# QEDProtocol/plonky2.5

Measured on AMD Instinct MI355X. Metric: recursive proofs/sec (fib-64 p3-in-p2 circuit), higher is better.
Workload: dtype u64 (Goldilocks, p = 2^64 - 2^32 + 1); 1 GPU; batch of 256 independent fib-64 plonky3-verifier proofs per GPU (n = 2^16 rows x 135 wires, LDE 2^19), 1 GPU(s), replicas + RCCL gather; all_statuses_ok=True, gathered_complete_and_ok=True, head=

## Files before the change

### plonky2.5_amd/csrc/kernels_ntt.hip

```cpp
#include <mutex>
#include <set>
#include <tuple>
#include "kernels.h"
#include "ntt16.h"

constexpr int NTT_FACTOR_LOG = 16;

namespace p25 {

template <int G>
__device__ __forceinline__ void dif_group(u64* col, const u64* wl, int step, int l, int lstride, int s0) {
  constexpr int K = 1 << G;
  u64 x[K];
#pragma unroll
  for (int k = 0; k < K; k++) x[k] = col[k * step];
#pragma unroll
  for (int m = 0; m < G; m++) {
    constexpr int dummy = 0;
    (void)dummy;
    const int hk = K >> (m + 1);
#pragma unroll
    for (int k = 0; k < K; k++) {
      if (k & hk) continue;
      const int j = ((k & (hk - 1)) << lstride) + l;
      u64 sum, d;
      gl::bfly_nc(x[k], x[k + hk], false, sum, d);
      x[k] = sum;
      x[k + hk] = (hk == 1 && lstride == 0) ? d : gl::mul_nc(d, wl[j << (s0 + m)]);
    }
  }
#pragma unroll
  for (int k = 0; k < K; k++) col[k * step] = x[k];
}

template <bool INV>
__device__ __forceinline__ void dif16_group(u64* col, const u64* wl, int step, int l, int s0) {
  u64 x[16];
#pragma unroll
  for (int k = 0; k < 16; k++) x[k] = col[k * step];
  dft16<INV>(x);
  if (l != 0) {
#pragma unroll
    for (int k = 1; k < 16; k++) {
      const int f = ((k & 1) << 3) | ((k & 2) << 1) | ((k & 4) >> 1) | ((k & 8) >> 3);
      x[k] = gl::mul_nc(x[k], wl[(l * f) << s0]);
    }
  }
#pragma unroll
  for (int k = 0; k < 16; k++) col[k * step] = x[k];
}

template <bool INV, int NTH, int PRE>
__global__ __launch_bounds__(NTH) void k_ntt_tile(NttPass a) {
  P25_WAVE_PRIO(P25_PRIO_BULK);
  extern __shared__ u64 lds[];
  const int R = 1 << a.log_r, T = 1 << a.log_t;
  const int TP = T > 1 ? T + 1 : 1;
  u64* wl = lds + (size_t)R * TP;
  const u32 NT = 1u << a.log_nt;
  const int tid = threadIdx.x, nth = blockDim.x;
  const int wstride_log = a.log_n_table - a.log_r;
  for (int k = tid; k < (a.full_table ? R : R / 2); k += nth) wl[k] = a.pow_table[(size_t)k << wstride_log];
  const u32 L = blockIdx.x;
  const u32 m = L >> a.log_g;
  const u32 tiles_g = a.n_tiles >> a.log_g;
  const u32 coset = m % a.n_cosets;
  const u32 r = m / a.n_cosets;
  const u32 tile = (r % tiles_g) * (1u << a.log_g) + (L & ((1u << a.log_g) - 1u));
  const u32 poly = r / tiles_g;
  const u32 tg0 = tile * T;
  const u64* in = a.in + (size_t)poly * a.in_poly_stride;
  u64* out = a.out + (size_t)poly * a.out_poly_stride + a.coset_out_off[coset];
  const u64* pre = PRE == 1 ? a.pre + ((size_t)coset << (a.log_r + a.log_nt)) : nullptr;
  const u64* pre_i = PRE == 2 ? a.pre_i + ((size_t)coset << a.log_r) : nullptr;
  const u64 pre_tv = PRE == 2 ? a.pre_t[((size_t)coset << a.log_nt) + tg0 + (tid & (T - 1))] : 1;
  auto in_slot = [&](int e, size_t& addr, int& slot, int& ii) {
    int t, i;
    if (a.in_kind == 0) {
      t = e & (T - 1);
      i = e >> a.log_t;
      u32 ipos = a.in_br_i ? gl::bitrev(i, a.log_r) : i;
      addr = (size_t)(tg0 + t) + (size_t)ipos * NT;
    } else {
      int off = e & (R - 1);
      t = e >> a.log_r;
      i = a.in_br_i ? (int)gl::bitrev(off, a.log_r) : off;
      u32 trow = a.in_br_t ? gl::bitrev(tg0 + t, a.log_nt) : tg0 + t;
      addr = (size_t)trow * R + off;
    }
    slot = i * TP + t;
    ii = i;
  };
  constexpr int LB = 8;
  int e = tid;
  for (; e + (LB - 1) * nth < T * R; e += LB * nth) {
    u64 xv[LB], pv[LB];
    int slot[LB];
#pragma unroll
    for (int k = 0; k < LB; k++) {
      size_t addr;
      int ii;
      in_slot(e + k * nth, addr, slot[k], ii);
      xv[k] = in[addr];
      if constexpr (PRE == 1) pv[k] = pre[addr];
      else if constexpr (PRE == 2) pv[k] = pre_i[ii];
      else pv[k] = 1;
    }
#pragma unroll
    for (int k = 0; k < LB; k++) {
      if constexpr (PRE == 1) lds[slot[k]] = gl::mul_nc(xv[k], pv[k]);
      else if constexpr (PRE == 2) lds[slot[k]] = gl::mul_nc(gl::mul_nc(xv[k], pre_tv), pv[k]);
      else lds[slot[k]] = xv[k];
    }
  }
  for (; e < T * R; e += nth) {
    size_t addr;
    int slot, ii;
    in_slot(e, addr, slot, ii);
    u64 x = in[addr];
    if constexpr (PRE == 1) x = gl::mul_nc(x, pre[addr]);
    if constexpr (PRE == 2) x = gl::mul_nc(gl::mul_nc(x, pre_tv), pre_i[ii]);
    lds[slot] = x;
  }
  __syncthreads();

  for (int s0 = 0; s0 < a.log_r;) {
    const int g = a.log_r - s0 < 4 ? a.log_r - s0 : 4;
    const int lstride = a.log_r - s0 - g;
    const int items = T << (a.log_r - g);
    for (int b = tid; b < items; b += nth) {
      const int t = b & (T - 1), q = b >> a.log_t;
      const int l = q & ((1 << lstride) - 1), h = q >> lstride;
      u64* col = lds + ((h << (a.log_r - s0)) + l) * TP + t;
      switch (g) {
        case 4:
          if (a.full_table)
            dif16_group<INV>(col, wl, TP << lstride, l, s0);
          else
            dif_group<4>(col, wl, TP << lstride, l, lstride, s0);
          break;
        case 3: dif_group<3>(col, wl, TP << lstride, l, lstride, s0); break;
        case 2: dif_group<2>(col, wl, TP << lstride, l, lstride, s0); break;
        default: dif_group<1>(col, wl, TP << lstride, l, lstride, s0); break;
      }
    }
    __syncthreads();
    s0 += g;
  }

  auto out_slot = [&](int e, size_t& addr, int& slot, u32& tw, u32& j) {
    int t, q;
    if (a.out_kind == 0) {
      t = e & (T - 1);
      q = e >> a.log_t;
      j = gl::bitrev(q, a.log_r);
      u32 ipos = a.out_br_i ? (u32)q : j;
      addr = (size_t)(tg0 + t) + (size_t)ipos * NT;
    } else {
      int off = e & (R - 1);
      t = e >> a.log_r;
      q = a.out_br_i ? off : (int)gl::bitrev(off, a.log_r);
      j = gl::bitrev(q, a.log_r);
      u32 trow = a.out_br_t ? gl::bitrev(tg0 + t, a.log_nt) : tg0 + t;
      addr = (size_t)trow * R + off;
    }
    slot = q * TP + t;
    tw = (u32)(tg0 + t);
  };
  int eo = tid;
  if (a.use_twiddle && !a.post_t) {
    for (; eo + (LB - 1) * nth < T * R; eo += LB * nth) {
      u64 wv[LB], xv[LB];
      size_t addr[LB];
#pragma unroll
      for (int k = 0; k < LB; k++) {
        int slot;
        u32 tw, j;
        out_slot(eo + k * nth, addr[k], slot, tw, j);
        wv[k] = a.pow_table[(size_t)tw * j];
        xv[k] = lds[slot];
      }
#pragma unroll
      for (int k = 0; k < LB; k++) {
        const u64 y = gl::mul_nc(xv[k], wv[k]);
        out[addr[k]] = a.lazy_out ? y : gl::canon(y);
      }
    }
  }
  for (; eo < T * R; eo += nth) {
    size_t addr;
    int slot;
    u32 tw, j;
    out_slot(eo, addr, slot, tw, j);
    u64 x = lds[slot];
    if (a.use_twiddle) x = gl::mul_nc(x, a.pow_table[(size_t)tw * j]);
    if (a.post_t) x = gl::mul_nc(x, gl::mul_nc(a.post_t[tw], a.post_i[j]));
    out[addr] = a.lazy_out ? x : gl::canon(x);
  }
}

static size_t tile_lds_bytes(int log_r, int log_t) {
  const size_t R = (size_t)1 << log_r, T = (size_t)1 << log_t, TP = T > 1 ? T + 1 : 1;
  return (R * TP + (log_r <= 10 ? R : R / 2)) * sizeof(u64);
}

void launch_ntt_pass(const NttPass& p, int n_polys, int n_cosets, hipStream_t st) {
  NttPass q = p;
  q.full_table = p.log_r <= 10;
  size_t lds = tile_lds_bytes(p.log_r, p.log_t);
  q.n_tiles = 1u << (p.log_nt - p.log_t);
  q.n_cosets = (uint32_t)n_cosets;
  q.log_g = 0;
  while (q.log_g < 3 && (2u << q.log_g) <= q.n_tiles) q.log_g++;
  const dim3 grid(q.n_tiles * (uint32_t)n_polys * (uint32_t)n_cosets);
  const bool wide = p.log_r + p.log_t >= 13;
  const int pre_mode = q.pre ? 1 : (q.pre_t ? 2 : 0);
  auto launch = [&](auto kernel, int nth) {
    if (lds > 64 * 1024) {
      static std::mutex mu;
      static std::set<std::pair<int, const void*>> allowed;
      int dev = 0;
      P25_HIP(hipGetDevice(&dev));
      std::lock_guard<std::mutex> lk(mu);
      if (allowed.insert({dev, (const void*)kernel}).second)
        P25_HIP(hipFuncSetAttribute((const void*)kernel, hipFuncAttributeMaxDynamicSharedMemorySize, 160 * 1024));
    }
    hipLaunchKernelGGL(kernel, grid, dim3(nth), lds, st, q);
  };
#define P25_NTT_LAUNCH(INV, NTH)                                                            \
  switch (pre_mode) {                                                                       \
    case 1: launch(k_ntt_tile<INV, NTH, 1>, NTH); break;                                    \
    case 2: launch(k_ntt_tile<INV, NTH, 2>, NTH); break;                                    \
    default: launch(k_ntt_tile<INV, NTH, 0>, NTH); break;                                   \
  }
  if (wide) {
    if (q.inverse) { P25_NTT_LAUNCH(true, 512) } else { P25_NTT_LAUNCH(false, 512) }
  } else {
    if (q.inverse) { P25_NTT_LAUNCH(true, 256) } else { P25_NTT_LAUNCH(false, 256) }
  }
#undef P25_NTT_LAUNCH
}

static int pick_log_t(int log_r, int log_nt, bool strided) {
  int lt = 12 - log_r;
  if (strided)
    for (int w = 4; w > lt; w--)
      if (tile_lds_bytes(log_r, w) <= 79 * 1024) {
        lt = w;
        break;
      }
  if (!strided && log_r == 10) lt = 3;
  if (lt > 4) lt = 4;
  if (lt > log_nt) lt = log_nt;
  if (lt < 0) lt = 0;
  return lt;
}

void ntt_inverse_then_lde(NttTables& tb, const u64* d_vals, size_t val_stride, u64* d_tmp, size_t tmp_stride, u64* d_coeffs,
                          size_t coeff_stride, u64* d_lde, size_t lde_stride, int log_n, int rate_bits, int n_polys, u64 shift,
                          hipStream_t st) {
  ntt_inverse(tb, d_vals, val_stride, false, d_tmp, tmp_stride, d_coeffs, coeff_stride, log_n, n_polys, 1, st);
  ntt_lde_bitrev(tb, d_coeffs, coeff_stride, d_lde, lde_stride, log_n, rate_bits, n_polys, shift, st);
}

const u64* NttTables::upload(const std::vector<u64>& host) {
  owned_.emplace_back(host.size());
  u64* d = owned_.back().p;
  P25_HIP(hipMemcpy(d, host.data(), host.size() * sizeof(u64), hipMemcpyHostToDevice));
  return d;
}
const u64* NttTables::pow_table(int log_n, bool inverse) {
  auto key = std::make_pair(log_n, inverse);
  auto it = pow_.find(key);
  if (it != pow_.end()) return it->second;
  u64 w = gl::root_of_unity(log_n);
  if (inverse) w = gl::inv(w);
  std::vector<u64> h((size_t)1 << log_n);
  u64 x = 1;
  for (auto& v : h) {
    v = x;
    x = gl::mul(x, w);
  }
  u64* d = const_cast<u64*>(upload(h));
  pow_[key] = d;
  return d;
}
const u64* NttTables::geom_table(u64 first, u64 ratio, size_t len) {
  auto key = std::make_tuple(first, ratio, len);
  auto it = geom_.find(key);
  if (it != geom_.end()) return it->second;
  std::vector<u64> h(len);
  u64 x = first;
  for (auto& v : h) {
    v = x;
    x = gl::mul(x, ratio);
  }
  u64* d = const_cast<u64*>(upload(h));
  geom_[key] = d;
  return d;
}

static void split(int log_n, int& log_r1, int& log_r2) {
  if (log_n <= 10) {
    log_r1 = 0;
    log_r2 = log_n;
  } else {
    log_r2 = log_n / 2;
    log_r1 = log_n - log_r2;
  }
  if (log_r1 > 11 || log_r2 > 11) throw std::runtime_error("NTT size above 2^22 not supported");
}

void ntt_inverse(NttTables& tb, const u64* d_in, size_t in_stride, bool in_bitrev, u64* d_tmp,
                 size_t tmp_stride, u64* d_out, size_t out_stride, int log_n, int n_polys,
                 u64 coset_shift, hipStream_t st) {
  int l1, l2;
  split(log_n, l1, l2);
  const u64* pw = tb.pow_table(log_n, true);
  u64 n_inv = gl::inv((u64)1 << log_n);
  u64 s_inv = gl::inv(coset_shift);
  NttPass p{};
  p.pow_table = pw;
  p.log_n_table = log_n;
  p.inverse = 1;
  if (l1 == 0) {
    p.in = d_in; p.out = d_out;
    p.in_poly_stride = in_stride; p.out_poly_stride = out_stride;
    p.log_r = l2; p.log_nt = 0; p.log_t = 0;
    p.in_kind = 1; p.in_br_i = in_bitrev;
    p.out_kind = 1; p.out_br_i = 0;
    p.post_t = tb.geom_table(n_inv, 1, 1);
    p.post_i = tb.geom_table(1, s_inv, (size_t)1 << l2);
    launch_ntt_pass(p, n_polys, 1, st);
    return;
  }
  p.in = d_in; p.out = d_tmp;
  p.in_poly_stride = in_stride; p.out_poly_stride = tmp_stride;
  p.log_r = l2; p.log_nt = l1; p.log_t = pick_log_t(l2, l1, true);
  if (in_bitrev) { p.in_kind = 1; p.in_br_t = 1; p.in_br_i = 1; } else { p.in_kind = 0; }
  p.out_kind = 0; p.out_br_i = 0;
  p.use_twiddle = 1;
  p.lazy_out = 1;
  launch_ntt_pass(p, n_polys, 1, st);
  NttPass q{};
  q.pow_table = pw; q.log_n_table = log_n;
  q.inverse = 1;
  q.in = d_tmp; q.out = d_out;
  q.in_poly_stride = tmp_stride; q.out_poly_stride = out_stride;
  q.log_r = l1; q.log_nt = l2; q.log_t = pick_log_t(l1, l2, false);
  q.in_kind = 1;
  q.out_kind = 0; q.out_br_i = 0;
  q.post_t = tb.geom_table(n_inv, s_inv, (size_t)1 << l2);
  q.post_i = tb.geom_table(1, gl::pow(s_inv, (u64)1 << l2), (size_t)1 << l1);
  launch_ntt_pass(q, n_polys, 1, st);
}

void ntt_lde_bitrev(NttTables& tb, const u64* d_coeffs, size_t coeff_stride, u64* d_lde,
                    size_t lde_stride, int log_n, int rate_bits, int n_polys, u64 shift,
                    hipStream_t st) {
  int l1, l2;
  split(log_n, l1, l2);
  const int nc = 1 << rate_bits;
  if (nc > 8) throw std::runtime_error("rate_bits > 3 not supported");
  const size_t n = (size_t)1 << log_n;
  const u64* pw = tb.pow_table(log_n, false);
  const u64 w_big = gl::root_of_unity(log_n + rate_bits);
  auto& cache = tb.coset_cache();
  const bool factored = l1 != 0 && log_n > NTT_FACTOR_LOG;
  auto key = std::make_tuple(factored ? -log_n : log_n, rate_bits, shift);
  auto it = cache.find(key);
  if (it == cache.end()) {
    std::vector<u64> h;
    if (!factored) {
      h.resize((size_t)nc * n);
      for (int c = 0; c < nc; c++) {
        u64 sc = gl::mul(shift, gl::pow(w_big, c));
        u64 x = 1;
        for (size_t k = 0; k < n; k++) {
          h[(size_t)c * n + k] = x;
          x = gl::mul(x, sc);
        }
      }
    } else {
      const size_t R1 = (size_t)1 << l1, R2 = (size_t)1 << l2;
      h.resize((size_t)nc * (R1 + R2));
      for (int c = 0; c < nc; c++) {
        const u64 sc = gl::mul(shift, gl::pow(w_big, c)), sc_r1 = gl::pow(sc, R1);
        u64 x = 1;
        for (size_t k = 0; k < R1; k++) {
          h[(size_t)c * R1 + k] = x;
          x = gl::mul(x, sc);
        }
        x = 1;
        for (size_t k = 0; k < R2; k++) {
          h[(size_t)nc * R1 + (size_t)c * R2 + k] = x;
          x = gl::mul(x, sc_r1);
        }
      }
    }
    it = cache.emplace(key, tb.upload(h)).first;
  }

  NttPass p{};
  p.pow_table = pw; p.log_n_table = log_n;
  p.in = d_coeffs; p.out = d_lde;
  p.in_poly_stride = coeff_stride; p.out_poly_stride = lde_stride;
  for (int c = 0; c < nc; c++) p.coset_out_off[c] = (size_t)gl::bitrev(c, rate_bits) * n;
  if (factored) {
    p.pre_t = it->second;
    p.pre_i = it->second + ((size_t)nc << l1);
  } else {
    p.pre = it->second;
  }
  if (l1 == 0) {
    p.log_r = l2; p.log_nt = 0; p.log_t = 0;
    p.in_kind = 1; p.out_kind = 1; p.out_br_i = 1;
    launch_ntt_pass(p, n_polys, nc, st);
    return;
  }
  p.log_r = l2; p.log_nt = l1; p.log_t = pick_log_t(l2, l1, true);
  p.in_kind = 0; p.out_kind = 0; p.out_br_i = 1;
  p.use_twiddle = 1;
  p.lazy_out = 1;
  launch_ntt_pass(p, n_polys, nc, st);
  NttPass q{};
  q.pow_table = pw; q.log_n_table = log_n;
  q.in = d_lde; q.out = d_lde;
  q.in_poly_stride = lde_stride; q.out_poly_stride = lde_stride;
  q.log_r = l1; q.log_nt = l2 + rate_bits; q.log_t = pick_log_t(l1, l2 + rate_bits, false);
  q.in_kind = 1; q.out_kind = 1; q.out_br_i = 1;
  launch_ntt_pass(q, n_polys, 1, st);
}

}
```

Baseline: 135.8 proofs/s.

## Specialize NTT tile kernel by access form with incremental index cursors

Replaces the runtime-branched index computation in the NTT tile kernel with template-specialized load/store cursors per input/output layout and multiplier mode, using 32-bit offsets and incremental stepping. Adds a fully compile-time stage network for the common log_r=8, log_t=4 shape, and precomputes twiddle pointers in the radix-16 group. The goal is to cut integer address arithmetic, branches and 64-bit index math in a hot kernel. In exchange it brings template bloat, 32-bit offsets that could overflow on large buffers, and a runtime throw for any pass form not in the list.

```diff
diff --git a/plonky2.5_amd/csrc/kernels_ntt.hip b/plonky2.5_amd/csrc/kernels_ntt.hip
--- a/plonky2.5_amd/csrc/kernels_ntt.hip
+++ b/plonky2.5_amd/csrc/kernels_ntt.hip
@@ -3,6 +3,7 @@
 #include <tuple>
 #include "kernels.h"
 #include "ntt16.h"
+#include "ntt_index.h"
 
 constexpr int NTT_FACTOR_LOG = 16;
 
@@ -33,169 +34,172 @@
   for (int k = 0; k < K; k++) col[k * step] = x[k];
 }
 
-template <bool INV>
+template <bool INV, int STEP>
 __device__ __forceinline__ void dif16_group(u64* col, const u64* wl, int step, int l, int s0) {
+  const int st = STEP > 0 ? STEP : step;
   u64 x[16];
 #pragma unroll
-  for (int k = 0; k < 16; k++) x[k] = col[k * step];
+  for (int k = 0; k < 16; k++) x[k] = col[k * st];
   dft16<INV>(x);
   if (l != 0) {
+    const u64* wf[16];
+    wf[0] = wl;
+#pragma unroll
+    for (int f = 1; f < 16; f++) wf[f] = wf[f - 1] + (l << s0);
 #pragma unroll
     for (int k = 1; k < 16; k++) {
       const int f = ((k & 1) << 3) | ((k & 2) << 1) | ((k & 4) >> 1) | ((k & 8) >> 3);
-      x[k] = gl::mul_nc(x[k], wl[(l * f) << s0]);
-    }
-  }
-#pragma unroll
-  for (int k = 0; k < 16; k++) col[k * step] = x[k];
-}
-
-template <bool INV, int NTH, int PRE>
+      x[k] = gl::mul_nc(x[k], *wf[f]);
+    }
+  }
+#pragma unroll
+  for (int k = 0; k < 16; k++) col[k * st] = x[k];
+}
+
+template <bool INV, bool FULL, int STEP>
+__device__ __forceinline__ void dif_stages(u64* lds, const u64* wl, int log_r, int log_t, int s0, int g, int tid, int nth) {
+  const int T = 1 << log_t, TP = (int)nttix::row_pitch(log_t);
+  const int lstride = log_r - s0 - g;
+  const int items = T << (log_r - g);
+  for (int b = tid; b < items; b += nth) {
+    const int t = b & (T - 1), q = b >> log_t;
+    const int l = q & ((1 << lstride) - 1), h = q >> lstride;
+    u64* col = lds + ((h << (log_r - s0)) + l) * TP + t;
+    switch (g) {
+      case 4:
+        if (FULL)
+          dif16_group<INV, STEP>(col, wl, TP << lstride, l, s0);
+        else
+          dif_group<4>(col, wl, TP << lstride, l, lstride, s0);
+        break;
+      case 3: dif_group<3>(col, wl, TP << lstride, l, lstride, s0); break;
+      case 2: dif_group<2>(col, wl, TP << lstride, l, lstride, s0); break;
+      default: dif_group<1>(col, wl, TP << lstride, l, lstride, s0); break;
+    }
+  }
+  __syncthreads();
+}
+template <bool INV, int NTH, int LR, int LT, int S0>
+__device__ __forceinline__ void dif_network_static(u64* lds, const u64* wl, int tid) {
+  if constexpr (S0 < LR) {
+    constexpr int g = LR - S0 < 4 ? LR - S0 : 4;
+    constexpr int TP = LT ? (1 << LT) + 1 : 1;
+    dif_stages<INV, (LR <= 10), (g == 4 ? TP << (LR - S0 - g) : 0)>(lds, wl, LR, LT, S0, g, tid, NTH);
+    dif_network_static<INV, NTH, LR, LT, S0 + g>(lds, wl, tid);
+  }
+}
+
+__device__ __forceinline__ u64 ld_w(const u64* base, u32 woff) {
+  return *reinterpret_cast<const u64*>(reinterpret_cast<const char*>(base) + (woff << 3));
+}
+__device__ __forceinline__ void st_w(u64* base, u32 woff, u64 v) {
+  *reinterpret_cast<u64*>(reinterpret_cast<char*>(base) + (woff << 3)) = v;
+}
+
+template <bool INV, int NTH, int PRE, int IN, int OUT, int MUL, bool LAZY, int LR, int LT>
 __global__ __launch_bounds__(NTH) void k_ntt_tile(NttPass a) {
   P25_WAVE_PRIO(P25_PRIO_BULK);
   extern __shared__ u64 lds[];
-  const int R = 1 << a.log_r, T = 1 << a.log_t;
-  const int TP = T > 1 ? T + 1 : 1;
+  const int log_r = LR >= 0 ? LR : a.log_r, log_t = LT >= 0 ? LT : a.log_t;
+  const int R = 1 << log_r, T = 1 << log_t;
+  const int TP = (int)nttix::row_pitch(log_t);
+  const int TR = T * R;
   u64* wl = lds + (size_t)R * TP;
-  const u32 NT = 1u << a.log_nt;
-  const int tid = threadIdx.x, nth = blockDim.x;
-  const int wstride_log = a.log_n_table - a.log_r;
-  for (int k = tid; k < (a.full_table ? R : R / 2); k += nth) wl[k] = a.pow_table[(size_t)k << wstride_log];
-  const u32 L = blockIdx.x;
-  const u32 m = L >> a.log_g;
-  const u32 tiles_g = a.n_tiles >> a.log_g;
-  const u32 coset = m % a.n_cosets;
-  const u32 r = m / a.n_cosets;
-  const u32 tile = (r % tiles_g) * (1u << a.log_g) + (L & ((1u << a.log_g) - 1u));
-  const u32 poly = r / tiles_g;
-  const u32 tg0 = tile * T;
-  const u64* in = a.in + (size_t)poly * a.in_poly_stride;
-  u64* out = a.out + (size_t)poly * a.out_poly_stride + a.coset_out_off[coset];
-  const u64* pre = PRE == 1 ? a.pre + ((size_t)coset << (a.log_r + a.log_nt)) : nullptr;
-  const u64* pre_i = PRE == 2 ? a.pre_i + ((size_t)coset << a.log_r) : nullptr;
-  const u64 pre_tv = PRE == 2 ? a.pre_t[((size_t)coset << a.log_nt) + tg0 + (tid & (T - 1))] : 1;
-  auto in_slot = [&](int e, size_t& addr, int& slot, int& ii) {
-    int t, i;
-    if (a.in_kind == 0) {
-      t = e & (T - 1);
-      i = e >> a.log_t;
-      u32 ipos = a.in_br_i ? gl::bitrev(i, a.log_r) : i;
-      addr = (size_t)(tg0 + t) + (size_t)ipos * NT;
-    } else {
-      int off = e & (R - 1);
-      t = e >> a.log_r;
-      i = a.in_br_i ? (int)gl::bitrev(off, a.log_r) : off;
-      u32 trow = a.in_br_t ? gl::bitrev(tg0 + t, a.log_nt) : tg0 + t;
-      addr = (size_t)trow * R + off;
-    }
-    slot = i * TP + t;
-    ii = i;
+  const int tid = threadIdx.x;
+  const int wstride_log = a.log_n_table - log_r;
+  const bool full_table = log_r <= 10;
+  for (int k = tid; k < (full_table ? R : R / 2); k += NTH) wl[k] = a.pow_table[(size_t)k << wstride_log];
+  const nttix::BlockId blk = nttix::decode_block(blockIdx.x, a.log_g, a.n_tiles, a.n_cosets);
+  const nttix::Tile tile{log_r, log_t, a.log_nt, blk.tile << log_t};
+  const u64* in = a.in + (size_t)blk.poly * a.in_poly_stride;
+  u64* out = a.out + (size_t)blk.poly * a.out_poly_stride + a.coset_out_off[blk.coset];
+  const u64* pre = PRE == 1 ? a.pre + ((size_t)blk.coset << (log_r + a.log_nt)) : nullptr;
+  const u64* pre_i = PRE == 2 ? a.pre_i + ((size_t)blk.coset << log_r) : nullptr;
+  const u64 pre_tv = PRE == 2 ? a.pre_t[((size_t)blk.coset << a.log_nt) + tile.tg0 + (tid & (T - 1))] : 1;
+  constexpr int LB = 8;
+  {
+    nttix::LoadCursor<IN> lc;
+    lc.init(tile, tid, NTH);
+    int e = tid;
+    for (; e + (LB - 1) * NTH < TR; e += LB * NTH) {
+      u64 xv[LB], pv[LB];
+      u32 slot[LB];
+#pragma unroll
+      for (int k = 0; k < LB; k++) {
+        const u32 g = lc.goff();
+        slot[k] = lc.slot();
+        xv[k] = ld_w(in, g);
+        if constexpr (PRE == 1) pv[k] = ld_w(pre, g);
+        else if constexpr (PRE == 2) pv[k] = pre_i[lc.idx()];
+        else pv[k] = 1;
+        lc.next();
+      }
+#pragma unroll
+      for (int k = 0; k < LB; k++) {
+        if constexpr (PRE == 1) lds[slot[k]] = gl::mul_nc(xv[k], pv[k]);
+        else if constexpr (PRE == 2) lds[slot[k]] = gl::mul_nc(gl::mul_nc(xv[k], pre_tv), pv[k]);
+        else lds[slot[k]] = xv[k];
+      }
+    }
+    for (; e < TR; e += NTH) {
+      const u32 g = lc.goff();
+      u64 x = ld_w(in, g);
+      if constexpr (PRE == 1) x = gl::mul_nc(x, ld_w(pre, g));
+      if constexpr (PRE == 2) x = gl::mul_nc(gl::mul_nc(x, pre_tv), pre_i[lc.idx()]);
+      lds[lc.slot()] = x;
+      lc.next();
+    }
+  }
+  __syncthreads();
+
+  if constexpr (LR >= 0) {
+    dif_network_static<INV, NTH, LR, LT, 0>(lds, wl, tid);
+  } else {
+    for (int s0 = 0; s0 < log_r;) {
+      const int g = log_r - s0 < 4 ? log_r - s0 : 4;
+      if (full_table)
+        dif_stages<INV, true, 0>(lds, wl, log_r, log_t, s0, g, tid, NTH);
+      else
+        dif_stages<INV, false, 0>(lds, wl, log_r, log_t, s0, g, tid, NTH);
+      s0 += g;
+    }
+  }
+
+  nttix::StoreCursor<OUT> sc;
+  sc.init(tile, tid, NTH);
+  constexpr bool T_KIND = OUT == nttix::OUT_T || OUT == nttix::OUT_T_BR;
+  const u64 post_tv = (MUL == nttix::MUL_POST && T_KIND) ? a.post_t[sc.tw()] : 1;
+  auto multiplier = [&](u64& w, u64& pt) {
+    if constexpr (MUL == nttix::MUL_TWIDDLE) w = ld_w(a.pow_table, __umul24(sc.tw(), sc.j()));
+    if constexpr (MUL == nttix::MUL_POST) {
+      w = a.post_i[sc.j()];
+      pt = T_KIND ? post_tv : a.post_t[sc.tw()];
+    }
   };
-  constexpr int LB = 8;
-  int e = tid;
-  for (; e + (LB - 1) * nth < T * R; e += LB * nth) {
-    u64 xv[LB], pv[LB];
-    int slot[LB];
-#pragma unroll
-    for (int k = 0; k < LB; k++) {
-      size_t addr;
-      int ii;
-      in_slot(e + k * nth, addr, slot[k], ii);
-      xv[k] = in[addr];
-      if constexpr (PRE == 1) pv[k] = pre[addr];
-      else if constexpr (PRE == 2) pv[k] = pre_i[ii];
-      else pv[k] = 1;
-    }
-#pragma unroll
-    for (int k = 0; k < LB; k++) {
-      if constexpr (PRE == 1) lds[slot[k]] = gl::mul_nc(xv[k], pv[k]);
-      else if constexpr (PRE == 2) lds[slot[k]] = gl::mul_nc(gl::mul_nc(xv[k], pre_tv), pv[k]);
-      else lds[slot[k]] = xv[k];
-    }
-  }
-  for (; e < T * R; e += nth) {
-    size_t addr;
-    int slot, ii;
-    in_slot(e, addr, slot, ii);
-    u64 x = in[addr];
-    if constexpr (PRE == 1) x = gl::mul_nc(x, pre[addr]);
-    if constexpr (PRE == 2) x = gl::mul_nc(gl::mul_nc(x, pre_tv), pre_i[ii]);
-    lds[slot] = x;
-  }
-  __syncthreads();
-
-  for (int s0 = 0; s0 < a.log_r;) {
-    const int g = a.log_r - s0 < 4 ? a.log_r - s0 : 4;
-    const int lstride = a.log_r - s0 - g;
-    const int items = T << (a.log_r - g);
-    for (int b = tid; b < items; b += nth) {
-      const int t = b & (T - 1), q = b >> a.log_t;
-      const int l = q & ((1 << lstride) - 1), h = q >> lstride;
-      u64* col = lds + ((h << (a.log_r - s0)) + l) * TP + t;
-      switch (g) {
-        case 4:
-          if (a.full_table)
-            dif16_group<INV>(col, wl, TP << lstride, l, s0);
-          else
-            dif_group<4>(col, wl, TP << lstride, l, lstride, s0);
-          break;
-        case 3: dif_group<3>(col, wl, TP << lstride, l, lstride, s0); break;
-        case 2: dif_group<2>(col, wl, TP << lstride, l, lstride, s0); break;
-        default: dif_group<1>(col, wl, TP << lstride, l, lstride, s0); break;
-      }
-    }
-    __syncthreads();
-    s0 += g;
-  }
-
-  auto out_slot = [&](int e, size_t& addr, int& slot, u32& tw, u32& j) {
-    int t, q;
-    if (a.out_kind == 0) {
-      t = e & (T - 1);
-      q = e >> a.log_t;
-      j = gl::bitrev(q, a.log_r);
-      u32 ipos = a.out_br_i ? (u32)q : j;
-      addr = (size_t)(tg0 + t) + (size_t)ipos * NT;
-    } else {
-      int off = e & (R - 1);
-      t = e >> a.log_r;
-      q = a.out_br_i ? off : (int)gl::bitrev(off, a.log_r);
-      j = gl::bitrev(q, a.log_r);
-      u32 trow = a.out_br_t ? gl::bitrev(tg0 + t, a.log_nt) : tg0 + t;
-      addr = (size_t)trow * R + off;
-    }
-    slot = q * TP + t;
-    tw = (u32)(tg0 + t);
+  auto finish = [&](u64 x, u64 w, u64 pt) {
+    if constexpr (MUL == nttix::MUL_TWIDDLE) x = gl::mul_nc(x, w);
+    if constexpr (MUL == nttix::MUL_POST) x = gl::mul_nc(x, gl::mul_nc(pt, w));
+    return LAZY ? x : gl::canon(x);
   };
   int eo = tid;
-  if (a.use_twiddle && !a.post_t) {
-    for (; eo + (LB - 1) * nth < T * R; eo += LB * nth) {
-      u64 wv[LB], xv[LB];
-      size_t addr[LB];
-#pragma unroll
-      for (int k = 0; k < LB; k++) {
-        int slot;
-        u32 tw, j;
-        out_slot(eo + k * nth, addr[k], slot, tw, j);
-        wv[k] = a.pow_table[(size_t)tw * j];
-        xv[k] = lds[slot];
-      }
-#pragma unroll
-      for (int k = 0; k < LB; k++) {
-        const u64 y = gl::mul_nc(xv[k], wv[k]);
-        out[addr[k]] = a.lazy_out ? y : gl::canon(y);
-      }
-    }
-  }
-  for (; eo < T * R; eo += nth) {
-    size_t addr;
-    int slot;
-    u32 tw, j;
-    out_slot(eo, addr, slot, tw, j);
-    u64 x = lds[slot];
-    if (a.use_twiddle) x = gl::mul_nc(x, a.pow_table[(size_t)tw * j]);
-    if (a.post_t) x = gl::mul_nc(x, gl::mul_nc(a.post_t[tw], a.post_i[j]));
-    out[addr] = a.lazy_out ? x : gl::canon(x);
+  for (; eo + (LB - 1) * NTH < TR; eo += LB * NTH) {
+    u64 wv[LB], ptv[LB], xv[LB];
+    u32 g[LB];
+#pragma unroll
+    for (int k = 0; k < LB; k++) {
+      g[k] = sc.goff();
+      multiplier(wv[k], ptv[k]);
+      xv[k] = lds[sc.slot()];
+      sc.next();
+    }
+#pragma unroll
+    for (int k = 0; k < LB; k++) st_w(out, g[k], finish(xv[k], wv[k], ptv[k]));
+  }
+  for (; eo < TR; eo += NTH) {
+    u64 w = 1, pt = 1;
+    multiplier(w, pt);
+    st_w(out, sc.goff(), finish(lds[sc.slot()], w, pt));
+    sc.next();
   }
 }
 
@@ -205,6 +209,7 @@
 }
 
 void launch_ntt_pass(const NttPass& p, int n_polys, int n_cosets, hipStream_t st) {
+  using namespace nttix;
   NttPass q = p;
   q.full_table = p.log_r <= 10;
   size_t lds = tile_lds_bytes(p.log_r, p.log_t);
@@ -214,6 +219,7 @@
   while (q.log_g < 3 && (2u << q.log_g) <= q.n_tiles) q.log_g++;
   const dim3 grid(q.n_tiles * (uint32_t)n_polys * (uint32_t)n_cosets);
   const bool wide = p.log_r + p.log_t >= 13;
+  const bool hot = p.log_r == 8 && p.log_t == 4;
   const int pre_mode = q.pre ? 1 : (q.pre_t ? 2 : 0);
   auto launch = [&](auto kernel, int nth) {
     if (lds > 64 * 1024) {
@@ -227,18 +233,36 @@
     }
     hipLaunchKernelGGL(kernel, grid, dim3(nth), lds, st, q);
   };
-#define P25_NTT_LAUNCH(INV, NTH)                                                            \
-  switch (pre_mode) {                                                                       \
-    case 1: launch(k_ntt_tile<INV, NTH, 1>, NTH); break;                                    \
-    case 2: launch(k_ntt_tile<INV, NTH, 2>, NTH); break;                                    \
-    default: launch(k_ntt_tile<INV, NTH, 0>, NTH); break;                                   \
-  }
-  if (wide) {
-    if (q.inverse) { P25_NTT_LAUNCH(true, 512) } else { P25_NTT_LAUNCH(false, 512) }
-  } else {
-    if (q.inverse) { P25_NTT_LAUNCH(true, 256) } else { P25_NTT_LAUNCH(false, 256) }
-  }
-#undef P25_NTT_LAUNCH
+  int in = -1, out = -1;
+  if (p.in_kind == 0 && !p.in_br_i) in = IN_T;
+  if (p.in_kind == 1 && !p.in_br_t && !p.in_br_i) in = IN_I;
+  if (p.in_kind == 1 && p.in_br_i && (p.in_br_t || p.log_nt == 0)) in = IN_I_BR;
+  if (!p.out_br_t) out = p.out_kind == 0 ? (p.out_br_i ? OUT_T_BR : OUT_T) : (p.out_br_i ? OUT_I_BR : OUT_I);
+  const int mul = p.post_t ? MUL_POST : (p.use_twiddle ? MUL_TWIDDLE : MUL_NONE);
+  const bool both = p.post_t && p.use_twiddle;
+#define P25_NTT_FORM(INV, PRE, IN, OUT, MUL, LAZY, WIDE, HOT)                                                         \
+  if (!both && (bool)q.inverse == INV && pre_mode == PRE && in == IN && out == OUT && mul == MUL && (bool)q.lazy_out == LAZY && \
+      (WIDE || !wide)) {                                                                                              \
+    if (wide) {                                                                                                       \
+      if constexpr (WIDE) launch(k_ntt_tile<INV, 512, PRE, IN, OUT, MUL, LAZY, -1, -1>, 512);                         \
+    } else if (HOT && hot) {                                                                                          \
+      if constexpr (HOT) launch(k_ntt_tile<INV, 256, PRE, IN, OUT, MUL, LAZY, 8, 4>, 256);                            \
+    } else {                                                                                                          \
+      launch(k_ntt_tile<INV, 256, PRE, IN, OUT, MUL, LAZY, -1, -1>, 256);                                             \
+    }                                                                                                                 \
+    return;                                                                                                           \
+  }
+  P25_NTT_FORM(true, 0, IN_T, OUT_T, MUL_TWIDDLE, true, true, true)
+  P25_NTT_FORM(true, 0, IN_I_BR, OUT_T, MUL_TWIDDLE, true, true, false)
+  P25_NTT_FORM(true, 0, IN_I, OUT_T, MUL_POST, false, true, true)
+  P25_NTT_FORM(true, 0, IN_I, OUT_I, MUL_POST, false, false, false)
+  P25_NTT_FORM(true, 0, IN_I_BR, OUT_I, MUL_POST, false, false, false)
+  P25_NTT_FORM(false, 1, IN_T, OUT_T_BR, MUL_TWIDDLE, true, true, true)
+  P25_NTT_FORM(false, 2, IN_T, OUT_T_BR, MUL_TWIDDLE, true, true, false)
+  P25_NTT_FORM(false, 0, IN_I, OUT_I_BR, MUL_NONE, false, true, true)
+  P25_NTT_FORM(false, 1, IN_I, OUT_I_BR, MUL_NONE, false, false, false)
+#undef P25_NTT_FORM
+  throw std::runtime_error("NTT pass of a form the library has no kernel for");
 }
 
 static int pick_log_t(int log_r, int log_nt, bool strided) {
diff --git a/plonky2.5_amd/csrc/ntt_index.h b/plonky2.5_amd/csrc/ntt_index.h
--- /dev/null
+++ b/plonky2.5_amd/csrc/ntt_index.h
@@ -0,0 +1,140 @@
+#pragma once
+#include <stdint.h>
+
+#if defined(__HIPCC__)
+#define NTTIX_HD __host__ __device__ __forceinline__
+#else
+#define NTTIX_HD inline
+#endif
+
+namespace p25 {
+namespace nttix {
+
+enum In : int {
+  IN_T = 0,
+  IN_I = 1,
+  IN_I_BR = 2,
+};
+enum Out : int {
+  OUT_T = 0,
+  OUT_T_BR = 1,
+  OUT_I = 2,
+  OUT_I_BR = 3,
+};
+enum Mul : int {
+  MUL_NONE = 0,
+  MUL_TWIDDLE = 1,
+  MUL_POST = 2,
+};
+
+struct Tile {
+  int log_r, log_t, log_nt;
+  uint32_t tg0;
+};
+
+NTTIX_HD uint32_t brev(uint32_t x, int bits) {
+#if defined(__HIP_DEVICE_COMPILE__)
+  return bits ? (__brev(x) >> (32 - bits)) : 0;
+#else
+  uint32_t r = 0;
+  for (int b = 0; b < bits; b++) r |= ((x >> b) & 1u) << (bits - 1 - b);
+  return r;
+#endif
+}
+NTTIX_HD uint32_t row_pitch(int log_t) { return log_t ? (1u << log_t) + 1u : 1u; }
+
+struct BlockId {
+  uint32_t tile, poly, coset;
+};
+NTTIX_HD BlockId decode_block(uint32_t L, uint32_t log_g, uint32_t n_tiles, uint32_t n_cosets) {
+  const uint32_t m = L >> log_g, tiles_g = n_tiles >> log_g;
+  const uint32_t r = m / n_cosets;
+  return BlockId{(r % tiles_g) * (1u << log_g) + (L & ((1u << log_g) - 1u)), r / tiles_g, m % n_cosets};
+}
+
+template <int IN>
+struct LoadCursor {
+  uint32_t g, s, i;
+  uint32_t dg, ds, di;
+  uint32_t e, de, base;
+  int log_r, log_nt;
+  uint32_t tp, tg0;
+
+  NTTIX_HD void init(const Tile& a, uint32_t tid, uint32_t nth) {
+    log_r = a.log_r, log_nt = a.log_nt, tp = row_pitch(a.log_t), tg0 = a.tg0;
+    if constexpr (IN == IN_T) {
+      const uint32_t t = tid & ((1u << a.log_t) - 1u);
+      i = tid >> a.log_t, di = nth >> a.log_t;
+      g = tg0 + t + (i << log_nt), dg = di << log_nt;
+      s = i * tp + t, ds = di * tp;
+    } else {
+      e = tid, de = nth, base = tg0 << log_r;
+    }
+  }
+  NTTIX_HD void next() {
+    if constexpr (IN == IN_T) g += dg, s += ds, i += di;
+    else e += de;
+  }
+  NTTIX_HD uint32_t idx() const {
+    if constexpr (IN == IN_T) return i;
+    const uint32_t off = e & ((1u << log_r) - 1u);
+    return IN == IN_I_BR ? brev(off, log_r) : off;
+  }
+  NTTIX_HD uint32_t slot() const {
+    if constexpr (IN == IN_T) return s;
+    return idx() * tp + (e >> log_r);
+  }
+  NTTIX_HD uint32_t goff() const {
+    if constexpr (IN == IN_T) return g;
+    if constexpr (IN == IN_I) return base + e;
+    return (brev(tg0 + (e >> log_r), log_nt) << log_r) + (e & ((1u << log_r) - 1u));
+  }
+};
+
+template <int OUT>
+struct StoreCursor {
+  uint32_t g, s, q;
+  uint32_t dg, ds, dq;
+  uint32_t e, de, base;
+  int log_r, log_nt;
+  uint32_t tp, tg0, twv;
+
+  NTTIX_HD void init(const Tile& a, uint32_t tid, uint32_t nth) {
+    log_r = a.log_r, log_nt = a.log_nt, tp = row_pitch(a.log_t), tg0 = a.tg0;
+    if constexpr (OUT == OUT_T || OUT == OUT_T_BR) {
+      const uint32_t t = tid & ((1u << a.log_t) - 1u);
+      twv = tg0 + t;
+      q = tid >> a.log_t, dq = nth >> a.log_t;
+      g = twv + (q << log_nt), dg = dq << log_nt;
+      s = q * tp + t, ds = dq * tp;
+    } else {
+      e = tid, de = nth, base = tg0 << log_r;
+    }
+  }
+  NTTIX_HD void next() {
+    if constexpr (OUT == OUT_T || OUT == OUT_T_BR) g += dg, s += ds, q += dq;
+    else e += de;
+  }
+  NTTIX_HD uint32_t tw() const {
+    if constexpr (OUT == OUT_T || OUT == OUT_T_BR) return twv;
+    return tg0 + (e >> log_r);
+  }
+  NTTIX_HD uint32_t j() const {
+    if constexpr (OUT == OUT_T || OUT == OUT_T_BR) return brev(q, log_r);
+    const uint32_t off = e & ((1u << log_r) - 1u);
+    return OUT == OUT_I_BR ? brev(off, log_r) : off;
+  }
+  NTTIX_HD uint32_t slot() const {
+    if constexpr (OUT == OUT_T || OUT == OUT_T_BR) return s;
+    const uint32_t off = e & ((1u << log_r) - 1u);
+    return (OUT == OUT_I_BR ? off : brev(off, log_r)) * tp + (e >> log_r);
+  }
+  NTTIX_HD uint32_t goff() const {
+    if constexpr (OUT == OUT_T_BR) return g;
+    if constexpr (OUT == OUT_T) return twv + (j() << log_nt);
+    return base + e;
+  }
+};
+
+}
+}
```

After: 139.5 proofs/s, median of 6. +2.7%, better.
